# tartarughina/S-BLAS

Hardware: AMD Instinct MI355X
Metric: SpMM GFLOP/s (2*nnz*N/t), CSR x dense N=64, fp64 (higher is better)
Workload: dtype f64; 1 GPU; SpMM method-1 (dense-B column partition), nd24k-like synthetic (M=K=72000, 399 nnz/row, band +-2000, seed 211), nnz=28728000, N=64 columns per GPU, alpha=beta=1, B = srand(211)/rand() as the reference's DenseMatrix, inputs resident in HBM; step = B->row-major staging + row-panel SpMM; rows=72000, cols=72000, nnz=28728000, n_cols_per_gpu=64, parallelism=method1-colblock x1

## Files before the change

include/sblas_hip.h:

```cpp
#ifndef SBLAS_HIP_H
#define SBLAS_HIP_H

#include <stddef.h>
#include <stdint.h>

#ifdef __cplusplus
extern "C" {
#endif

#define SBLAS_OK 0
#define SBLAS_E_INVALID 1
#define SBLAS_E_HIP 2
#define SBLAS_E_WORKSPACE 3
#define SBLAS_E_RCCL 4
#define SBLAS_E_IO 5
#define SBLAS_E_NOGPU 6

int sblas_hip_version(void);
const char *sblas_hip_error_string(int code);
int sblas_hip_device_count(void);

size_t sblas_hip_spmm_csr_f64_i32_workspace(int64_t rows, int64_t cols, int64_t nnz, int64_t n);

int sblas_hip_spmm_csr_f64_i32(int dev, void *stream,
// ... 255 lines not shown
    SBLAS_SPMM_RULE_STAGING = 0,
    SBLAS_SPMM_RULE_VERDICTS,
    SBLAS_SPMM_RULE_PANEL_ROWS,
    SBLAS_SPMM_RULE_GROUPS,
    SBLAS_SPMM_RULE_PANELS,
    SBLAS_SPMM_RULE_PLANNABLE,
    SBLAS_SPMM_RULE_TILED,
    SBLAS_SPMM_RULE_TILED_G,
    SBLAS_SPMM_RULE_W6_NH,
    SBLAS_SPMM_RULE_W6_GRID_Y,
    SBLAS_SPMM_RULE_LANES_NC,
    SBLAS_SPMM_RULE_LANES_CP,
    SBLAS_SPMM_RULE_LANES_LPE,
    SBLAS_SPMM_RULE_MFMA,
    SBLAS_SPMM_RULE_MFMA_BATCH,
    SBLAS_SPMM_RULE_MFMA_LDS_FLOOR,
    SBLAS_SPMM_RULE_FOUR_ROWS,
    SBLAS_SPMM_RULE_FOUR_ROWS_WAVES,
    SBLAS_SPMM_RULE_FOUR_ROWS_VOTED,
    SBLAS_SPMM_RULE_MERGE,
    SBLAS_SPMM_RULE_DPP_GROUPS,
    SBLAS_SPMM_RULE_DPP_PAD,
    SBLAS_SPMM_RULE_DPP_LONG,
    SBLAS_SPMM_RULE_NARROW,
    SBLAS_SPMM_RULE_ROWS8,
    SBLAS_SPMM_RULE_INTERLEAVE,
    SBLAS_SPMM_RULE_SKIP,
    SBLAS_SPMM_RULE_SPLIT_GROUPS,
    SBLAS_SPMM_RULE_FIELDS
};
int64_t sblas_spmm_rule_describe(int64_t rows, int64_t cols, int64_t nnz, int64_t ldbt, int64_t n, int64_t ncu,
                                 int caller_staged, const int64_t *plan, int64_t *out, int64_t max_out);

int sblas_host_fill_rand0to1(double *dst, int64_t count, unsigned seed);

int sblas_mm_read_info(const char *path, int32_t *rows, int32_t *cols, int32_t *nnz,
                       int32_t *is_symmetric);
int sblas_mm_read_csr(const char *path, int32_t *rowptr, int32_t *colidx, double *val);

#ifdef __cplusplus
}
#endif
#endif
```

s-blas_amd/csrc/kernels.hip:

```cpp
#include <hip/hip_runtime.h>
#include <atomic>
#include <stdint.h>
#include <algorithm>
#include <type_traits>
#include <mutex>
#include <vector>
#include "kernels.h"

namespace sblas {

constexpr int WAVE = 64;

__device__ __forceinline__ int wave_uniform(int v) { return __builtin_amdgcn_readfirstlane(v); }

__device__ __forceinline__ double readlane_f64(double v, int src_lane)
{
    int lo = __double2loint(v), hi = __double2hiint(v);
    lo = __builtin_amdgcn_readlane(lo, src_lane);
    hi = __builtin_amdgcn_readlane(hi, src_lane);
    return __hiloint2double(hi, lo);
}

constexpr int STAGE_K = 32;
template <bool RB>
__device__ __forceinline__ void stage_tile(double (*tile)[STAGE_K + 1], int64_t k0, int64_t j0, int64_t cols, int64_t n,
                                           const double *__restrict__ B, int64_t ldb, double *__restrict__ Bt,
                                           int64_t ldbt, int *__restrict__ tail, int stage_epoch)
{
    if constexpr (RB) {
        const int jl = threadIdx.x & 63, kq = threadIdx.x >> 6;
        const int64_t j = j0 + jl;
        double v[8];
#pragma unroll
        for (int u = 0; u < 8; ++u) {
            const int64_t kr = k0 + kq + 4 * u;
            v[u] = (j < n && kr < cols) ? B[kr * ldb + j] : 0.0;
        }
        bool odd = false;
#pragma unroll
        for (int u = 0; u < 8; ++u) odd |= (__double2hiint(v[u]) & 0x7ff00000) == 0x7ff00000;
// ... 577 lines not shown
                 "v_fmac_f64_dpp %[c3], %[gv], v[110:111] row_newbcast:" #K1 " row_mask:0xf bank_mask:0xf\n\t"       \
                 "s_waitcnt lgkmcnt(3)\n\t"                                                                          \
                 "v_fmac_f64_dpp %[c0], %[gv], v[112:113] row_newbcast:" #K2 " row_mask:0xf bank_mask:0xf\n\t"       \
                 "v_fmac_f64_dpp %[c1], %[gv], v[114:115] row_newbcast:" #K2 " row_mask:0xf bank_mask:0xf\n\t"       \
                 "s_waitcnt lgkmcnt(2)\n\t"                                                                          \
                 "v_fmac_f64_dpp %[c2], %[gv], v[116:117] row_newbcast:" #K2 " row_mask:0xf bank_mask:0xf\n\t"       \
                 "v_fmac_f64_dpp %[c3], %[gv], v[118:119] row_newbcast:" #K2 " row_mask:0xf bank_mask:0xf\n\t"       \
                 "s_waitcnt lgkmcnt(1)\n\t"                                                                          \
                 "v_fmac_f64_dpp %[c0], %[gv], v[120:121] row_newbcast:" #K3 " row_mask:0xf bank_mask:0xf\n\t"       \
                 "v_fmac_f64_dpp %[c1], %[gv], v[122:123] row_newbcast:" #K3 " row_mask:0xf bank_mask:0xf\n\t"       \
                 "s_waitcnt lgkmcnt(0)\n\t"                                                                          \
                 "v_fmac_f64_dpp %[c2], %[gv], v[124:125] row_newbcast:" #K3 " row_mask:0xf bank_mask:0xf\n\t"       \
                 "v_fmac_f64_dpp %[c3], %[gv], v[126:127] row_newbcast:" #K3 " row_mask:0xf bank_mask:0xf\n\t"       \
                 : [c0] "+v"(q0), [c1] "+v"(q1), [c2] "+v"(q2), [c3] "+v"(q3)                                        \
                 : [co] "v"(co), [lb] "v"(lb), [gv] "v"(gv)                                                          \
                 : "memory", "v92", "v93", "v94", "v95", "v96", "v97", "v98", "v99", "v100", "v101", "v102", "v103", \
                   "v104", "v105", "v106", "v107", "v108", "v109", "v110", "v111", "v112", "v113", "v114", "v115",   \
                   "v116", "v117", "v118", "v119", "v120", "v121", "v122", "v123", "v124", "v125", "v126", "v127")

__device__ __forceinline__ void dma_rows_scalar(unsigned lds_addr, unsigned voff, const char *base)
{
    asm volatile("s_mov_b32 m0, %0\n\ts_nop 0\n\tglobal_load_lds_dwordx4 %1, %2" ::"s"(lds_addr), "v"(voff), "s"(base)
                 : "memory");
}
__device__ __forceinline__ void dma_rows_vector(unsigned lds_addr, const char *addr)
{
    asm volatile("s_mov_b32 m0, %0\n\ts_nop 0\n\tglobal_load_lds_dwordx4 %1, off" ::"s"(lds_addr), "v"(addr)
                 : "memory");
}

static_assert(4 * 4 * 2 >= SPMM_MIN_PANEL_ROWS, "the workspace reserves one verdict per SPMM_MIN_PANEL_ROWS rows");


__device__ __forceinline__ void window_select6(int wc, double wv, int tile_lo, int rem, int k, unsigned zero_rel,
                                               unsigned &co, double &gv, unsigned long long &m)
{
    int glo, ghi;
    asm volatile("v_subrev_u32 %[co], %[tlo], %[wc]\n\t"
                 "v_cmp_gt_i32 %[m], %[rem], %[k]\n\t"
                 "v_cmp_gt_u32 vcc, %[tr], %[co]\n\t"
                 "v_lshlrev_b32 %[co], 9, %[co]\n\t"
                 "s_and_b64 vcc, vcc, %[m]\n\t"
                 "s_mov_b64 %[m], vcc\n\t"
                 "v_cndmask_b32 %[co], %[zr], %[co], vcc\n\t"
                 "v_cndmask_b32 %[glo], 0, %[vlo], vcc\n\t"
                 "v_cndmask_b32 %[ghi], 0, %[vhi], vcc"
                 : [co] "=&v"(co), [m] "=&s"(m), [glo] "=&v"(glo), [ghi] "=&v"(ghi)
                 : [tlo] "s"(tile_lo), [wc] "v"(wc), [rem] "v"(rem), [k] "v"(k), [zr] "v"(zero_rel),
                   [vlo] "v"(__double2loint(wv)), [vhi] "v"(__double2hiint(wv)), [tr] "n"(W2_ROWS)
                 : "vcc", "scc");
    gv = __hiloint2double(ghi, glo);
}
__device__ __forceinline__ void window_issue6(sblas_rsrc_t rc, sblas_rsrc_t rv, int idx, int &ca, double &va, int &cb,
                                              double &vb)
{
    const int idx2 = idx + 16;
    asm volatile("buffer_load_dword %0, %4, %6, 0 idxen\n\t"
                 "buffer_load_dwordx2 %1, %4, %7, 0 idxen\n\t"
                 "buffer_load_dword %2, %5, %6, 0 idxen\n\t"
                 "buffer_load_dwordx2 %3, %5, %7, 0 idxen"
                 : "=&v"(ca), "=&v"(va), "=&v"(cb), "=&v"(vb)
                 : "v"(idx), "v"(idx2), "s"(rc), "s"(rv)
                 : "memory");
}
template <int NEWER> __device__ __forceinline__ void window_wait6(int &ca, double &va, int &cb, double &vb)
{
    static_assert(NEWER == 0 || NEWER == 4 || NEWER == 8, "counts of the sixth-generation tile loop");
    if (NEWER == 4) asm volatile("s_waitcnt vmcnt(4)" : "+v"(ca), "+v"(va), "+v"(cb), "+v"(vb)::"memory");
    else if (NEWER == 8) asm volatile("s_waitcnt vmcnt(8)" : "+v"(ca), "+v"(va), "+v"(cb), "+v"(vb)::"memory");
    else asm volatile("s_waitcnt vmcnt(0)" : "+v"(ca), "+v"(va), "+v"(cb), "+v"(vb)::"memory");
}
template <int N> __device__ __forceinline__ void vm_wait6()
{
    static_assert(N == 8 || N == 12, "counts of the sixth-generation tile loop");
    if (N == 12) asm volatile("s_waitcnt vmcnt(12)" ::: "memory");
    else asm volatile("s_waitcnt vmcnt(8)" ::: "memory");
}

template <int G, int NH, bool RC>
__global__ __launch_bounds__(1024) void spmm_window6_kernel(
    int rows, int cols, int npanels, const int *__restrict__ rowptr, const int *__restrict__ colidx,
    const double *__restrict__ val, const double *__restrict__ Bt, int64_t ldbt, int n, double alpha, double beta,
    double *__restrict__ C, int64_t ldc, const int *__restrict__ tail, const int2 *__restrict__ info,
    const int *__restrict__ cls, int panel_rows, int nnz)
{
    constexpr int RW = 4 * G, RMAX = 16 * RW;
    static_assert(G == 2 || G == 3, "two or three groups per wave (the counted vmcnt waits are 4 G)");
    static_assert(NH == 1 || NH == 2, "one or two 64-column halves per workgroup");
    static_assert(64 * (RMAX + 1) <= 2 * W2_TILE, "C tile must fit in the (dead) B tile buffers");
    extern __shared__ __attribute__((aligned(16))) double smem[];
    double *zero_row = smem + 2 * W2_TILE;
    int *sm_i = reinterpret_cast<int *>(smem + 2 * W2_TILE + 64);

    const int panel = xcd_contiguous_panel(blockIdx.x, npanels);
    if (!owns_window(tail, cls, panel)) return;
    const int2 span = info[panel];

    const int tid = threadIdx.x;
    const int lane = tid & 63;
    const int wave = wave_uniform(tid >> 6);
    const int row0 = panel * panel_rows;
    const int col0 = blockIdx.y * (64 * NH);
    const unsigned ld32 = (unsigned)ldbt;
    const int t_lo = span.x / W2_ROWS, t_hi = span.y / W2_ROWS;
    const bool loader = wave >= 12;
    const bool active = !loader && wave * RW < panel_rows;

    if (tid < 64) zero_row[tid] = 0.0;
    if (tid == 0) sm_i[0] = 0;

    double acc[NH][G][4];
#pragma unroll
    for (int h = 0; h < NH; ++h)
#pragma unroll
        for (int g = 0; g < G; ++g)
#pragma unroll
            for (int j = 0; j < 4; ++j) acc[h][g][j] = 0.0;

    const unsigned ldb8 = ld32 * 8u;
    const unsigned piece_off = (unsigned)(col0 + ((lane & 31) << 1)) * 8u;
    const unsigned pair_off = (unsigned)(lane >> 5) * ldb8 + piece_off;
    const char *bt_bytes = reinterpret_cast<const char *>(Bt);
    int dummy = 0;
    auto dma_part = [&](int t, int h, int buf) {
        const int lw = wave - 12;
        const int r0 = t * W2_ROWS + lw * W2_LROWS;
        const unsigned lds0 = (unsigned)wave_uniform((int)((unsigned)(uintptr_t)(smem + buf * W2_TILE) + (unsigned)lw * (unsigned)(W2_LROWS * 512)));
        const unsigned hoff = (unsigned)h * 512u;
        if (r0 + W2_LROWS - 1 <= cols) {
            const char *p = bt_bytes + (size_t)((unsigned)r0 * ldb8) + hoff;
#pragma unroll
            for (int i = 0; i < W2_LROWS / 2; ++i) dma_rows_scalar(lds0 + i * 1024u, pair_off, p + (size_t)(2u * i) * ldb8);
        } else {
#pragma unroll
            for (int i = 0; i < W2_LROWS / 2; ++i) {
                const unsigned brow = (unsigned)min(r0 + 2 * i + (lane >> 5), cols);
                dma_rows_vector(lds0 + i * 1024u, bt_bytes + (size_t)(brow * ldb8 + piece_off + hoff));
            }
        }
    };

    if (loader) dma_part(t_lo, 0, 0);

    const int k = lane & 15, q = lane >> 4;
    const int wrow = min(row0 + wave * RW, rows);
    const int wstart = wave_uniform(rowptr[wrow]);
    const sblas_rsrc_t rc = make_rsrc(colidx + wstart, 4u, (unsigned)(nnz - wstart));
    const sblas_rsrc_t rv = make_rsrc(val + wstart, 8u, (unsigned)(nnz - wstart));
    int cur[G], end[G];
#pragma unroll
    for (int g = 0; g < G; ++g) {
        const int rr = wave * RW + 4 * g + q;
        const int row = row0 + rr;
        cur[g] = end[g] = 0;
        if (rr < panel_rows && row < rows) {
            cur[g] = rowptr[row] - wstart;
            end[g] = rowptr[row + 1] - wstart;
        }
    }
    unsigned long long viol = 0ull;
    int wca[G], wcb[G];
    double wva[G], wvb[G];
    unsigned s_coA[G], s_coB[G];
    double s_gvA[G], s_gvB[G];
    int s_take[G], s_mx[G];
    bool replay[G];
#pragma unroll
    for (int g = 0; g < G; ++g) {
        s_coA[g] = s_coB[g] = 0u;
        s_gvA[g] = s_gvB[g] = 0.0;
        s_take[g] = s_mx[g] = 0;
        replay[g] = false;
    }
#pragma unroll
    for (int g = 0; g < G; ++g) window_issue6(rc, rv, cur[g] + k, wca[g], wva[g], wcb[g], wvb[g]);
    asm volatile("s_waitcnt vmcnt(0)" ::: "memory");
    __syncthreads();
    int step = 0;
    for (int t = t_lo; t <= t_hi; ++t) {
        const int tile_lo = t * W2_ROWS;
        auto half = [&](auto hc) {
            constexpr int h = decltype(hc)::value;
            const int cbuf = step & 1;
            if (loader) {
                if (h + 1 < NH) dma_part(t, h + 1, cbuf ^ 1);
                else if (t < t_hi) dma_part(t + 1, 0, cbuf ^ 1);
            }
            const unsigned tile_base = (unsigned)(uintptr_t)(smem + cbuf * W2_TILE);
            const unsigned lb = tile_base + (unsigned)k * 16u;
            const unsigned zero_rel = (unsigned)(uintptr_t)zero_row - tile_base;
            auto visit = [&](auto gc) {
                constexpr int g = decltype(gc)::value;
                if (h == 0) window_wait6<NH == 1 ? 4 * (G - 1) : 4 * (G - 1 - g)>(wca[g], wva[g], wcb[g], wvb[g]);
                else if (replay[g]) window_wait6<0>(wca[g], wva[g], wcb[g], wvb[g]);
                double &q0 = acc[h][g][0], &q1 = acc[h][g][1], &q2 = acc[h][g][2], &q3 = acc[h][g][3];
                int lc = cur[g];
                bool full = h == 0 || replay[g];
                for (;;) {
                    unsigned coA, coB;
                    double gvA, gvB;
                    int take, mx;
                    if (full) {
                        const int rem = end[g] - lc;
                        unsigned long long mA, mB;
                        window_select6(wca[g], wva[g], tile_lo, rem, k, zero_rel, coA, gvA, mA);
                        window_select6(wcb[g], wvb[g], tile_lo, rem - 16, k, zero_rel, coB, gvB, mB);
                        const unsigned fa = q < 2 ? (unsigned)mA : (unsigned)(mA >> 32);
                        const unsigned fb = q < 2 ? (unsigned)mB : (unsigned)(mB >> 32);
                        const int sh = (q & 1) * 16;
                        take = __popc((fa >> sh) & 0xffffu) + __popc((fb >> sh) & 0xffffu);
                        viol |= mA ^ __builtin_amdgcn_ballot_w64(k < take);
                        viol |= mB ^ __builtin_amdgcn_ballot_w64(k + 16 < take);
                        mx = max(max(__builtin_amdgcn_readlane(take, 0), __builtin_amdgcn_readlane(take, 16)),
                                 max(__builtin_amdgcn_readlane(take, 32), __builtin_amdgcn_readlane(take, 48)));
                        if (NH > 1 && h == 0) {
                            s_coA[g] = coA, s_coB[g] = coB, s_gvA[g] = gvA, s_gvB[g] = gvB, s_take[g] = take, s_mx[g] = mx;
// ... 5 lines not shown
                    {
                        const unsigned co = coA;
                        const double gv = gvA;
                        if (mx > 0) { SBLAS_QSTEP4(0, 1, 2, 3); }
                        if (mx > 4) { SBLAS_QSTEP4(4, 5, 6, 7); }
                        if (mx > 8) { SBLAS_QSTEP4(8, 9, 10, 11); }
                        if (mx > 12) { SBLAS_QSTEP4(12, 13, 14, 15); }
                    }
                    if (mx > 16) {
                        const unsigned co = coB;
                        const double gv = gvB;
                        SBLAS_QSTEP4(0, 1, 2, 3);
                        if (mx > 20) { SBLAS_QSTEP4(4, 5, 6, 7); }
                        if (mx > 24) { SBLAS_QSTEP4(8, 9, 10, 11); }
                        if (mx > 28) { SBLAS_QSTEP4(12, 13, 14, 15); }
                    }
                    asm volatile("s_setprio 0" ::: "memory");
                    lc += take;
                    const bool more = take >= 32 && lc < end[g];
                    if (__builtin_expect(__builtin_amdgcn_ballot_w64(more) == 0ull, 1)) break;
                    if (NH > 1 && h == 0) replay[g] = true;
                    window_issue6(rc, rv, lc + k, wca[g], wva[g], wcb[g], wvb[g]);
                    window_wait6<0>(wca[g], wva[g], wcb[g], wvb[g]);
                    full = true;
                }
                if (h == NH - 1) {
                    cur[g] = lc;
                    if (NH > 1) replay[g] = false;
                    window_issue6(rc, rv, cur[g] + k, wca[g], wva[g], wcb[g], wvb[g]);
                } else if (replay[g]) {
                    window_issue6(rc, rv, cur[g] + k, wca[g], wva[g], wcb[g], wvb[g]);
                }
            };
            if (active) {
                visit(std::integral_constant<int, 0>{});
                visit(std::integral_constant<int, 1>{});
                if constexpr (G > 2) visit(std::integral_constant<int, 2>{});
            }
            if (loader) asm volatile("s_waitcnt vmcnt(0)" : "+v"(dummy)::"memory");
            __syncthreads();
            ++step;
        };
        half(std::integral_constant<int, 0>{});
        if constexpr (NH > 1) half(std::integral_constant<int, 1>{});
    }
#pragma unroll
    for (int g = 0; g < G; ++g) window_wait6<0>(wca[g], wva[g], wcb[g], wvb[g]);
    int bad = viol != 0ull ? 1 : 0;
#pragma unroll
    for (int g = 0; g < G; ++g)
        if (__builtin_amdgcn_ballot_w64(cur[g] < end[g]) != 0ull) bad = 1;
    if (bad && lane == 0) atomicOr(&sm_i[0], 1);
    __syncthreads();
    const bool fell_back = sm_i[0] != 0;
    if (tid == 0 && blockIdx.y == 0) atomicAdd(&g_panel_stats[fell_back ? 2 : 0], 1ull);

    double *ctile = smem;
    const int nrows = min(panel_rows, rows - row0);
#pragma unroll
    for (int h = 0; h < NH; ++h) {
        const int colh = col0 + 64 * h;
        if (fell_back) {
            const unsigned lane_off = (unsigned)(colh + lane);
#pragma unroll
            for (int g = 0; g < G; ++g)
#pragma unroll
                for (int j = 0; j < 4; ++j) {
                    const int rr = wave * RW + 4 * g + j;
                    const int row = row0 + rr;
                    int a = 0, b = 0;
// ... 1574 lines not shown
```

s-blas_amd/csrc/spmm_rule.cpp:

```cpp
#include <stdint.h>
#include <stdio.h>
#include <stdlib.h>
#include <string.h>
#include <algorithm>
#include <atomic>
#include <mutex>
#include "../../include/sblas_hip.h"
#include "kernels.h"

namespace sblas {

static Options g_options;
static std::atomic<bool> g_options_loaded{false};
static std::mutex g_options_mu;
static void options_parse(Options &o)
{
    o = Options{};
    const char *e;
    if ((e = getenv("SBLAS_SPMM_VARIANT")) && *e) {
        if (!strcmp(e, "dpp")) o.spmm_variant = SPMM_VARIANT_DIRECT_DPP;
        else if (!strcmp(e, "rows")) o.spmm_variant = SPMM_VARIANT_DIRECT_ROWS;
        else if (!strcmp(e, "lanes")) o.spmm_variant = SPMM_VARIANT_LANES;
        else if (!strcmp(e, "merge")) o.spmm_variant = SPMM_VARIANT_DIRECT_MERGE;
        else if (!strcmp(e, "mfma")) o.spmm_variant = SPMM_VARIANT_MFMA;
        else if (!strcmp(e, "nomfma")) o.spmm_variant = SPMM_VARIANT_NO_MFMA;
    }
    if ((e = getenv("SBLAS_SPMV_VARIANT")) && *e && strcmp(e, "auto")) {
        strncpy(o.spmv_variant, e, sizeof o.spmv_variant - 1);
    }
    if ((e = getenv("SBLAS_SPMM_MIN_LDBT")) && *e) o.tier16 = o.tier32 = atoi(e) < 64;
    if ((e = getenv("SBLAS_SPMM_MAX_BT_BYTES")) && *e) {
        const unsigned long long v = strtoull(e, nullptr, 10);
        if (v >= 4096 && v < 0xffffffffull) o.max_bt_bytes = v;
    }
    if ((e = getenv("SBLAS_DIRECT_LDS")) && *e) o.direct_lds = atoi(e);
    if ((e = getenv("SBLAS_DIRECT_MERGE")) && *e) o.direct_merge = atoi(e);
    if ((e = getenv("SBLAS_STAGE_RANGE")) && *e) o.stage_range = atoi(e);
    if ((e = getenv("SBLAS_DIRECT_MAP")) && *e) o.direct_map = !strcmp(e, "interleave") ? 1 : !strcmp(e, "contiguous") ? 0 : -1;
    if ((e = getenv("SBLAS_ROWS8_MIN_AVG")) && *e) o.rows8_min_avg = atof(e);
    if ((e = getenv("SBLAS_WINDOW_DENSITY")) && *e) o.window_density = (float)atof(e);
    if ((e = getenv("SBLAS_SPMM_PANEL_ROWS")) && *e) {
// ... 277 lines not shown
        pv.n_window = (long)plan[SBLAS_SPMM_RULE_PLAN_N_WINDOW], pv.n_direct = (long)plan[SBLAS_SPMM_RULE_PLAN_N_DIRECT];
        pv.n_mfma_w = (long)plan[SBLAS_SPMM_RULE_PLAN_N_MFMA_W], pv.n_mfma_d = (long)plan[SBLAS_SPMM_RULE_PLAN_N_MFMA_D];
        pv.merge = plan[SBLAS_SPMM_RULE_PLAN_MERGE] != 0, pv.four_rows = plan[SBLAS_SPMM_RULE_PLAN_FOUR_ROWS] != 0;
        pv.n_split = plan[SBLAS_SPMM_RULE_PLAN_N_SPLIT];
        pv.info_rows = (int)plan[SBLAS_SPMM_RULE_PLAN_PANEL_ROWS], pv.groups = (int)plan[SBLAS_SPMM_RULE_PLAN_GROUPS];
    }
    bool again = false;
    const sblas::SpmmStep st = sblas::step_rule((int)rows, (int)cols, nnz, ldbt, plan ? &pv : nullptr, sblas::SpmmStep(),
                                                caller_staged != 0, (int)ncu, again);
    const sblas::SpmmStage2 d = sblas::spmm_stage2(st, (int)rows, (int)cols, nnz, (int)n);
    int64_t f[SBLAS_SPMM_RULE_FIELDS] = {0};
    f[SBLAS_SPMM_RULE_STAGING] = st.staging, f[SBLAS_SPMM_RULE_VERDICTS] = st.verdicts;
    f[SBLAS_SPMM_RULE_PANEL_ROWS] = st.info_rows, f[SBLAS_SPMM_RULE_GROUPS] = st.groups;
    f[SBLAS_SPMM_RULE_PANELS] = st.npanels, f[SBLAS_SPMM_RULE_PLANNABLE] = st.plannable;
    f[SBLAS_SPMM_RULE_TILED] = d.tiled, f[SBLAS_SPMM_RULE_TILED_G] = d.tiled ? d.g : 0;
    f[SBLAS_SPMM_RULE_W6_NH] = d.nh, f[SBLAS_SPMM_RULE_W6_GRID_Y] = d.grid_y;
    f[SBLAS_SPMM_RULE_LANES_NC] = d.nc, f[SBLAS_SPMM_RULE_LANES_CP] = d.cp, f[SBLAS_SPMM_RULE_LANES_LPE] = d.lpe;
    f[SBLAS_SPMM_RULE_MFMA] = d.mfma;
    f[SBLAS_SPMM_RULE_MFMA_BATCH] = d.mfma ? d.mfma_batch : 0;
    f[SBLAS_SPMM_RULE_MFMA_LDS_FLOOR] = d.mfma ? (int64_t)d.mfma_lds_floor : 0;
    f[SBLAS_SPMM_RULE_FOUR_ROWS] = d.four_rows;
    f[SBLAS_SPMM_RULE_FOUR_ROWS_WAVES] = d.four_rows ? d.rows_waves : 0;
    f[SBLAS_SPMM_RULE_FOUR_ROWS_VOTED] = d.voted;
    f[SBLAS_SPMM_RULE_MERGE] = d.merge;
    f[SBLAS_SPMM_RULE_DPP_GROUPS] = d.dpp;
    f[SBLAS_SPMM_RULE_DPP_PAD] = d.dpp ? (int64_t)d.dpp_pad : 0;
    f[SBLAS_SPMM_RULE_DPP_LONG] = d.dpp ? d.dpp_long : 0;
    f[SBLAS_SPMM_RULE_NARROW] = d.narrow, f[SBLAS_SPMM_RULE_ROWS8] = d.rows8;
    f[SBLAS_SPMM_RULE_INTERLEAVE] = d.interleave;
    f[SBLAS_SPMM_RULE_SKIP] = d.skip, f[SBLAS_SPMM_RULE_SPLIT_GROUPS] = d.skip ? d.split_groups : 0;
    for (int64_t k = 0; out && k < SBLAS_SPMM_RULE_FIELDS && k < max_out; ++k) out[k] = f[k];
    return SBLAS_SPMM_RULE_FIELDS;
}
```

s-blas_amd/python/sblas_amd/__init__.py:

```python
import ctypes as C
import os

import numpy as np

_PKG = os.path.dirname(os.path.abspath(__file__))
_ROOT = os.path.normpath(os.path.join(_PKG, "..", ".."))
LIB_PATH = os.environ.get("SBLAS_LIB_PATH") or os.path.join(_ROOT, "lib", "libsblas_hip.so")

EXPORTS = [
    "sblas_hip_version", "sblas_hip_error_string", "sblas_hip_device_count",
    "sblas_hip_spmm_csr_f64_i32_workspace", "sblas_hip_spmm_csr_f64_i32", "sblas_hip_spmm_ldbt",
    "sblas_hip_dense_to_rowmajor_f64", "sblas_hip_spmm_csr_rowmajorB_f64_i32",
    "sblas_hip_debug_spmm_panel_stats", "sblas_hip_debug_reload_env",
    "sblas_hip_debug_spmm_kernel_events", "sblas_hip_debug_spmm_last_kernel_ms", "sblas_hip_spmv_csr_f64_i32", "sblas_hip_axpby_f64",
    "sblas_hip_comm_get", "sblas_hip_comm_release_all", "sblas_hip_allreduce_sum_f64",
    "sblas_hip_merge_rowblocks_f64", "sblas_hip_merge_rowblocks_local_f64",
    "sblas_find_row_of_nnz", "sblas_partition_nnz", "sblas_partition_dense",
    "sblas_mm_read_info", "sblas_mm_read_csr", "sblas_host_fill_rand0to1",
    "sblas_hip_spmm_csr_workspace", "sblas_hip_spmm_csr", "sblas_hip_spmv_csr", "sblas_hip_axpby",
    "sblas_hip_allreduce_sum", "sblas_hip_merge_rowblocks", "sblas_partition_nnz_i64",
    "sblas_hip_debug_validate_csr_i32",
    "sblas_hip_spmm_plan_create", "sblas_hip_spmm_plan_destroy", "sblas_hip_spmm_plan_info", "sblas_hip_spmm_csr_f64_i32_planned",
    "sblas_hip_spmv_plan_create", "sblas_hip_spmv_plan_destroy", "sblas_hip_spmv_plan_info", "sblas_hip_spmv_csr_f64_i32_planned",
    "sblas_spmv_plan_classify",
    "sblas_hip_spmm_csr_ordered", "sblas_hip_spmm_csr_ordered_f64_i32_planned", "sblas_hip_merge_rowblocks_ordered",
    "sblas_hip_spmm_plan_create_split", "sblas_hip_spmm_plan_split_info", "sblas_spmm_split_classify",
    "sblas_spmm_rule_describe",
    "sblas_hip_csr_transpose_workspace", "sblas_hip_csr_transpose_f64_i32", "sblas_hip_gather_f64",
    "sblas_hip_transpose_plan_create", "sblas_hip_transpose_plan_update_values", "sblas_hip_transpose_plan_info",
    "sblas_hip_transpose_plan_csc", "sblas_hip_transpose_plan_destroy", "sblas_hip_spmv_csr_t_f64_i32_planned",
    "sblas_hip_spmm_csr_t_f64_i32_planned",
    "sblas_hip_coo_to_csr_workspace", "sblas_hip_coo_to_csr_f64_i32", "sblas_hip_coo_plan_create", "sblas_hip_coo_plan_info",
    "sblas_hip_coo_plan_csr", "sblas_hip_coo_plan_assemble", "sblas_hip_coo_plan_destroy",
    "sblas_hip_sddmm_csr_workspace", "sblas_hip_sddmm_csr_f64_i32",
    "sblas_hip_csr_softmax_workspace", "sblas_hip_csr_softmax_f64_i32", "sblas_hip_csr_softmax_backward_f64_i32",
    "sblas_hip_csr_attention_workspace", "sblas_hip_csr_attention_f64_i32", "sblas_hip_csr_attention_backward_f64_i32",
    "sblas_hip_spgemm_limits", "sblas_hip_spgemm_classify", "sblas_hip_spgemm_group_width", "sblas_hip_spgemm_check_nnz",
    "sblas_hip_spgemm_plan_create", "sblas_hip_spgemm_plan_info", "sblas_hip_spgemm_plan_csr", "sblas_hip_spgemm_plan_numeric",
    "sblas_hip_spgemm_plan_destroy",
    "sblas_hip_sptrsv_limits", "sblas_sptrsv_levels", "sblas_sptrsv_schedule",
    "sblas_hip_sptrsv_plan_create", "sblas_hip_sptrsv_plan_info", "sblas_hip_sptrsv_plan_order", "sblas_hip_sptrsv_plan_destroy",
    "sblas_hip_sptrsv_f64_i32_planned", "sblas_hip_sptrsm_f64_i32_planned",
]


class SblasError(RuntimeError):
    pass


_lib = None


def lib():
    global _lib
    if _lib is not None:
        return _lib
    if not os.path.exists(LIB_PATH):
        raise SblasError("libsblas_hip.so not built (%s): run __graft_entry__.build() / make -C s-blas_amd" % LIB_PATH)
    import torch
    L = C.CDLL(LIB_PATH)
    i64, i32, f64, vp, sz = C.c_int64, C.c_int32, C.c_double, C.c_void_p, C.c_size_t
    L.sblas_hip_version.restype = C.c_int
    L.sblas_hip_error_string.restype = C.c_char_p
    L.sblas_hip_error_string.argtypes = [C.c_int]
    L.sblas_hip_device_count.restype = C.c_int
    L.sblas_hip_spmm_ldbt.restype = i64
    L.sblas_hip_spmm_ldbt.argtypes = [i64]
    L.sblas_hip_spmm_csr_f64_i32_workspace.restype = sz
    L.sblas_hip_spmm_csr_f64_i32_workspace.argtypes = [i64, i64, i64, i64]
    L.sblas_hip_spmm_csr_f64_i32.restype = C.c_int
    L.sblas_hip_spmm_csr_f64_i32.argtypes = [C.c_int, vp, i64, i64, i64, vp, vp, vp, vp, i64, i64, f64, f64, vp, i64, vp, sz]
    L.sblas_hip_debug_validate_csr_i32.restype = C.c_int
    L.sblas_hip_debug_validate_csr_i32.argtypes = [C.c_int, vp, i64, i64, i64, vp, vp]
    L.sblas_hip_spmm_plan_create.restype = C.c_int
    L.sblas_hip_spmm_plan_create.argtypes = [C.c_int, vp, i64, i64, i64, vp, vp, i64, C.POINTER(vp)]
    L.sblas_hip_spmm_plan_create_split.restype = C.c_int
    L.sblas_hip_spmm_plan_create_split.argtypes = [C.c_int, vp, i64, i64, i64, vp, vp, i64, i64, i64, C.POINTER(vp)]
    L.sblas_hip_spmm_plan_split_info.restype = C.c_int
    L.sblas_hip_spmm_plan_split_info.argtypes = [vp, C.POINTER(i64)]
    L.sblas_spmm_split_classify.restype = i64
    L.sblas_spmm_split_classify.argtypes = [vp, i64, i64, i64, i64, vp, i64, vp, i64]
    L.sblas_spmm_rule_describe.restype = i64
    L.sblas_spmm_rule_describe.argtypes = [i64, i64, i64, i64, i64, i64, C.c_int, vp, vp, i64]
    L.sblas_hip_spmm_plan_destroy.restype = C.c_int
    L.sblas_hip_spmm_plan_destroy.argtypes = [vp]
    L.sblas_hip_spmm_plan_info.restype = C.c_int
    L.sblas_hip_spmm_plan_info.argtypes = [vp, C.POINTER(i64)]
    L.sblas_hip_spmm_csr_f64_i32_planned.restype = C.c_int
    L.sblas_hip_spmm_csr_f64_i32_planned.argtypes = [vp, C.c_int, vp, i64, i64, i64, vp, vp, vp, vp, i64, i64, f64, f64, vp, i64, vp, sz]
    L.sblas_hip_spmv_plan_create.restype = C.c_int
    L.sblas_hip_spmv_plan_create.argtypes = [C.c_int, vp, i64, i64, i64, vp, vp, C.POINTER(vp)]
    L.sblas_hip_spmv_plan_destroy.restype = C.c_int
    L.sblas_hip_spmv_plan_destroy.argtypes = [vp]
    L.sblas_hip_spmv_plan_info.restype = C.c_int
    L.sblas_hip_spmv_plan_info.argtypes = [vp, C.POINTER(i64)]
    L.sblas_hip_spmv_csr_f64_i32_planned.restype = C.c_int
    L.sblas_hip_spmv_csr_f64_i32_planned.argtypes = [vp, C.c_int, vp, i64, i64, i64, vp, vp, vp, vp, f64, f64, vp]
    L.sblas_spmv_plan_classify.restype = i64
    L.sblas_spmv_plan_classify.argtypes = [vp, i64, i64, i64, i64, vp, i64]
    L.sblas_hip_dense_to_rowmajor_f64.restype = C.c_int
    L.sblas_hip_dense_to_rowmajor_f64.argtypes = [C.c_int, vp, i64, i64, vp, i64, vp, i64]
    L.sblas_hip_spmm_csr_rowmajorB_f64_i32.restype = C.c_int
    L.sblas_hip_spmm_csr_rowmajorB_f64_i32.argtypes = [C.c_int, vp, i64, i64, i64, vp, vp, vp, vp, i64, i64, f64, f64, vp, i64]
    L.sblas_hip_debug_reload_env.restype = C.c_int
    L.sblas_hip_debug_reload_env.argtypes = []
    L.sblas_hip_debug_spmm_panel_stats.restype = C.c_int
    L.sblas_hip_debug_spmm_panel_stats.argtypes = [C.POINTER(C.c_uint64), C.c_int]
    L.sblas_hip_debug_spmm_kernel_events.restype = C.c_int
    L.sblas_hip_debug_spmm_kernel_events.argtypes = [C.c_int]
    L.sblas_hip_debug_spmm_last_kernel_ms.restype = C.c_int
    L.sblas_hip_debug_spmm_last_kernel_ms.argtypes = [C.POINTER(C.c_float)]
    L.sblas_hip_spmv_csr_f64_i32.restype = C.c_int
    L.sblas_hip_spmv_csr_f64_i32.argtypes = [C.c_int, vp, i64, i64, i64, vp, vp, vp, vp, f64, f64, vp]
    L.sblas_hip_axpby_f64.restype = C.c_int
    L.sblas_hip_axpby_f64.argtypes = [C.c_int, vp, i64, f64, vp, f64, vp]
    L.sblas_hip_comm_get.restype = C.c_int
# ... 321 lines not shown

def sptrsv_schedule(widths, mode="auto", chain_rows=0):
    widths = np.ascontiguousarray(widths, np.int64)
    L = len(widths)
    kind = np.zeros(max(L, 1), np.uint8)
    first = np.zeros(L + 1, np.int64)
    n = C.c_int64()
    check(lib().sblas_sptrsv_schedule(L, widths.ctypes.data, _sptrsv_mode(mode), int(chain_rows), kind.ctypes.data,
                                      first.ctypes.data, C.byref(n)), "sblas_sptrsv_schedule")
    return kind[:n.value].copy(), first[:n.value + 1].copy()


def partition_dense(first_order, n_gpu, i_gpu):
    o, d = C.c_int64(), C.c_int64()
    check(lib().sblas_partition_dense(first_order, n_gpu, i_gpu, C.byref(o), C.byref(d)), "sblas_partition_dense")
    return o.value, d.value


def _dev_ptr(t, dtype, what):
    import torch
    if not isinstance(t, torch.Tensor) or not t.is_cuda:
        raise SblasError("%s must be a GPU tensor (no CPU path exists)" % what)
    if t.dtype != dtype or not t.is_contiguous():
        raise SblasError("%s must be a contiguous %s tensor" % (what, dtype))
    return t.data_ptr()


def _stream(stream=None):
    import torch
    s = stream if stream is not None else torch.cuda.current_stream()
    return C.c_void_p(s.cuda_stream)


def spmm_workspace_bytes(rows, cols, nnz, n):
    return int(lib().sblas_hip_spmm_csr_f64_i32_workspace(rows, cols, nnz, n))


def spmm(rows, cols, rowptr, colidx, val, B, ldb, n, alpha, beta, Cmat, ldc, workspace, stream=None, c_offset=0):
    import torch
    nnz = int(colidx.numel())
    rc = lib().sblas_hip_spmm_csr_f64_i32(
        -1, _stream(stream), rows, cols, nnz,
        _dev_ptr(rowptr, torch.int32, "rowptr"), _dev_ptr(colidx, torch.int32, "colidx") if nnz else None,
        _dev_ptr(val, torch.float64, "val") if nnz else None,
        _dev_ptr(B, torch.float64, "B") if cols else None, ldb, n, alpha, beta,
        _dev_ptr(Cmat, torch.float64, "C") + 8 * c_offset, ldc,
        _dev_ptr(workspace, torch.float64, "workspace") if workspace is not None and workspace.numel() else None,
        workspace.numel() * 8 if workspace is not None else 0)
    check(rc, "sblas_hip_spmm_csr_f64_i32")


class SpmmPlan:

    def __init__(self, rows, cols, rowptr, colidx, n, stream=None, split=False, split_min=0, piece=0):
        import torch
        self.rows, self.cols, self.n, self.rowptr, self.colidx = rows, cols, n, rowptr, colidx
        self.nnz = int(colidx.numel())
        h = C.c_void_p()
        args = (-1, _stream(stream), rows, cols, self.nnz, _dev_ptr(rowptr, torch.int32, "rowptr"),
                _dev_ptr(colidx, torch.int32, "colidx") if self.nnz else None, n)
        if split:
            check(lib().sblas_hip_spmm_plan_create_split(*args, split_min, piece, C.byref(h)), "sblas_hip_spmm_plan_create_split")
        else:
            check(lib().sblas_hip_spmm_plan_create(*args, C.byref(h)), "sblas_hip_spmm_plan_create")
        self.handle = h

# ... 1090 lines not shown
```

Baseline: 15050 GFLOP/s.

## Add aligned three-chunk ring buffer for colidx/val window loads in window6 kernel

For the single-half (NH==1) window6 kernel, colidx/val loads move from a sliding window at cur+k to a three-chunk ring aligned to the val pointer's 128-byte phase. Chunks already consumed are shifted in registers and only the newly needed chunks are fetched. The aim is cache-line-aligned, non-redundant nonzero loads across B tiles. The cost is a wider per-tile select and mask path (three selects per group), plus a possible refetch loop with a full vmcnt(0) wait. A host replay function is added to validate the ring logic.

```diff
diff --git a/include/sblas_hip.h b/include/sblas_hip.h
--- a/include/sblas_hip.h
+++ b/include/sblas_hip.h
@@ -311,6 +311,9 @@
 int64_t sblas_spmm_rule_describe(int64_t rows, int64_t cols, int64_t nnz, int64_t ldbt, int64_t n, int64_t ncu,
                                  int caller_staged, const int64_t *plan, int64_t *out, int64_t max_out);
 
+int64_t sblas_window_ring_replay(int64_t nnz, int64_t phase, int64_t cur, int64_t end, const int64_t *takes, int64_t ntakes,
+                                 int64_t *out, int64_t max_out, int64_t *stats);
+
 int sblas_host_fill_rand0to1(double *dst, int64_t count, unsigned seed);
 
 int sblas_mm_read_info(const char *path, int32_t *rows, int32_t *cols, int32_t *nnz,
diff --git a/s-blas_amd/csrc/kernels.hip b/s-blas_amd/csrc/kernels.hip
--- a/s-blas_amd/csrc/kernels.hip
+++ b/s-blas_amd/csrc/kernels.hip
@@ -6,6 +6,7 @@
 #include <mutex>
 #include <vector>
 #include "kernels.h"
+#include "window_ring.h"
 
 namespace sblas {
 
@@ -649,25 +650,29 @@
 static_assert(4 * 4 * 2 >= SPMM_MIN_PANEL_ROWS, "the workspace reserves one verdict per SPMM_MIN_PANEL_ROWS rows");
 
 
+#define SBLAS_SELECT6(CMP)                                                                                            \
+    asm volatile("v_subrev_u32 %[co], %[tlo], %[wc]\n\t" CMP " %[m], %[rem], %[k]\n\t"                               \
+                 "v_cmp_gt_u32 vcc, %[tr], %[co]\n\t"                                                                 \
+                 "v_lshlrev_b32 %[co], 9, %[co]\n\t"                                                                  \
+                 "s_and_b64 vcc, vcc, %[m]\n\t"                                                                       \
+                 "s_mov_b64 %[m], vcc\n\t"                                                                            \
+                 "v_cndmask_b32 %[co], %[zr], %[co], vcc\n\t"                                                         \
+                 "v_cndmask_b32 %[glo], 0, %[vlo], vcc\n\t"                                                           \
+                 "v_cndmask_b32 %[ghi], 0, %[vhi], vcc"                                                                \
+                 : [co] "=&v"(co), [m] "=&s"(m), [glo] "=&v"(glo), [ghi] "=&v"(ghi)                                    \
+                 : [tlo] "s"(tile_lo), [wc] "v"(wc), [rem] "v"(rem), [k] "v"(k), [zr] "v"(zero_rel),                   \
+                   [vlo] "v"(__double2loint(wv)), [vhi] "v"(__double2hiint(wv)), [tr] "n"(W2_ROWS)                     \
+                 : "vcc", "scc")
+template <bool RING = false>
 __device__ __forceinline__ void window_select6(int wc, double wv, int tile_lo, int rem, int k, unsigned zero_rel,
                                                unsigned &co, double &gv, unsigned long long &m)
 {
     int glo, ghi;
-    asm volatile("v_subrev_u32 %[co], %[tlo], %[wc]\n\t"
-                 "v_cmp_gt_i32 %[m], %[rem], %[k]\n\t"
-                 "v_cmp_gt_u32 vcc, %[tr], %[co]\n\t"
-                 "v_lshlrev_b32 %[co], 9, %[co]\n\t"
-                 "s_and_b64 vcc, vcc, %[m]\n\t"
-                 "s_mov_b64 %[m], vcc\n\t"
-                 "v_cndmask_b32 %[co], %[zr], %[co], vcc\n\t"
-                 "v_cndmask_b32 %[glo], 0, %[vlo], vcc\n\t"
-                 "v_cndmask_b32 %[ghi], 0, %[vhi], vcc"
-                 : [co] "=&v"(co), [m] "=&s"(m), [glo] "=&v"(glo), [ghi] "=&v"(ghi)
-                 : [tlo] "s"(tile_lo), [wc] "v"(wc), [rem] "v"(rem), [k] "v"(k), [zr] "v"(zero_rel),
-                   [vlo] "v"(__double2loint(wv)), [vhi] "v"(__double2hiint(wv)), [tr] "n"(W2_ROWS)
-                 : "vcc", "scc");
+    if constexpr (RING) SBLAS_SELECT6("v_cmp_gt_u32");
+    else SBLAS_SELECT6("v_cmp_gt_i32");
     gv = __hiloint2double(ghi, glo);
 }
+#undef SBLAS_SELECT6
 __device__ __forceinline__ void window_issue6(sblas_rsrc_t rc, sblas_rsrc_t rv, int idx, int &ca, double &va, int &cb,
                                               double &vb)
 {
@@ -694,6 +699,55 @@
     else asm volatile("s_waitcnt vmcnt(8)" ::: "memory");
 }
 
+__device__ __forceinline__ void ring_issue_all(sblas_rsrc_t rc, sblas_rsrc_t rv, int e0, int &c0, double &v0, int &c1,
+                                               double &v1, int &c2, double &v2)
+{
+    const int e1 = e0 + ring::CHUNK, e2 = e0 + 2 * ring::CHUNK;
+    asm volatile("buffer_load_dword %0, %6, %9, 0 idxen\n\t"
+                 "buffer_load_dwordx2 %1, %6, %10, 0 idxen\n\t"
+                 "buffer_load_dword %2, %7, %9, 0 idxen\n\t"
+                 "buffer_load_dwordx2 %3, %7, %10, 0 idxen\n\t"
+                 "buffer_load_dword %4, %8, %9, 0 idxen\n\t"
+                 "buffer_load_dwordx2 %5, %8, %10, 0 idxen"
+                 : "=&v"(c0), "=&v"(v0), "=&v"(c1), "=&v"(v1), "=&v"(c2), "=&v"(v2)
+                 : "v"(e0), "v"(e1), "v"(e2), "s"(rc), "s"(rv)
+                 : "memory");
+}
+__device__ __forceinline__ void ring_wait_all(int &c0, double &v0, int &c1, double &v1, int &c2, double &v2)
+{
+    asm volatile("s_waitcnt vmcnt(0)" : "+v"(c0), "+v"(v0), "+v"(c1), "+v"(v1), "+v"(c2), "+v"(v2)::"memory");
+}
+__device__ __forceinline__ void ring_advance(sblas_rsrc_t rc, sblas_rsrc_t rv, int e1, int e2, int n, int &c0, double &v0,
+                                             int &c1, double &v1, int &c2, double &v2)
+{
+    unsigned long long all;
+    asm volatile("s_mov_b64 %[all], exec\n\t"
+                 "v_cmp_lt_u32 vcc, 0, %[n]\n\t"
+                 "s_mov_b64 exec, vcc\n\t"
+                 "v_mov_b32 %[c0], %[c1]\n\t"
+                 "v_mov_b64 %[v0], %[v1]\n\t"
+                 "v_cmp_eq_u32 vcc, 1, %[n]\n\t"
+                 "s_mov_b64 exec, vcc\n\t"
+                 "v_mov_b32 %[c1], %[c2]\n\t"
+                 "v_mov_b64 %[v1], %[v2]\n\t"
+                 "s_mov_b64 exec, %[all]\n\t"
+                 "v_cmp_eq_u32 vcc, 2, %[n]\n\t"
+                 "s_mov_b64 exec, vcc\n\t"
+                 "v_mov_b32 %[c0], %[c2]\n\t"
+                 "v_mov_b64 %[v0], %[v2]\n\t"
+                 "buffer_load_dword %[c1], %[e1], %[rc], 0 idxen\n\t"
+                 "buffer_load_dwordx2 %[v1], %[e1], %[rv], 0 idxen\n\t"
+                 "s_mov_b64 exec, %[all]\n\t"
+                 "v_cmp_lt_u32 vcc, 0, %[n]\n\t"
+                 "s_mov_b64 exec, vcc\n\t"
+                 "buffer_load_dword %[c2], %[e2], %[rc], 0 idxen\n\t"
+                 "buffer_load_dwordx2 %[v2], %[e2], %[rv], 0 idxen\n\t"
+                 "s_mov_b64 exec, %[all]"
+                 : [all] "=&s"(all), [c0] "+v"(c0), [v0] "+v"(v0), [c1] "+v"(c1), [v1] "+v"(v1), [c2] "+v"(c2), [v2] "+v"(v2)
+                 : [e1] "v"(e1), [e2] "v"(e2), [n] "v"(n), [rc] "s"(rc), [rv] "s"(rv)
+                 : "memory", "vcc");
+}
+
 template <int G, int NH, bool RC>
 __global__ __launch_bounds__(1024) void spmm_window6_kernel(
     int rows, int cols, int npanels, const int *__restrict__ rowptr, const int *__restrict__ colidx,
@@ -702,6 +756,7 @@
     const int *__restrict__ cls, int panel_rows, int nnz)
 {
     constexpr int RW = 4 * G, RMAX = 16 * RW;
+    constexpr bool RING = NH == 1;
     static_assert(G == 2 || G == 3, "two or three groups per wave (the counted vmcnt waits are 4 G)");
     static_assert(NH == 1 || NH == 2, "one or two 64-column halves per workgroup");
     static_assert(64 * (RMAX + 1) <= 2 * W2_TILE, "C tile must fit in the (dead) B tile buffers");
@@ -761,9 +816,10 @@
 
     const int k = lane & 15, q = lane >> 4;
     const int wrow = min(row0 + wave * RW, rows);
-    const int wstart = wave_uniform(rowptr[wrow]);
+    const int wstart = RING ? 0 : wave_uniform(rowptr[wrow]);
     const sblas_rsrc_t rc = make_rsrc(colidx + wstart, 4u, (unsigned)(nnz - wstart));
     const sblas_rsrc_t rv = make_rsrc(val + wstart, 8u, (unsigned)(nnz - wstart));
+    const int phase = wave_uniform(ring::phase((uint64_t)(uintptr_t)val));
     int cur[G], end[G];
 #pragma unroll
     for (int g = 0; g < G; ++g) {
@@ -778,6 +834,8 @@
     unsigned long long viol = 0ull;
     int wca[G], wcb[G];
     double wva[G], wvb[G];
+    int wc0[G], re0[G];
+    double wv0[G];
     unsigned s_coA[G], s_coB[G];
     double s_gvA[G], s_gvB[G];
     int s_take[G], s_mx[G];
@@ -790,7 +848,19 @@
         replay[g] = false;
     }
 #pragma unroll
-    for (int g = 0; g < G; ++g) window_issue6(rc, rv, cur[g] + k, wca[g], wva[g], wcb[g], wvb[g]);
+    for (int g = 0; g < G; ++g) {
+        if constexpr (RING) {
+            re0[g] = ring::r0_entry(cur[g], phase, k);
+            ring_issue_all(rc, rv, re0[g], wc0[g], wv0[g], wca[g], wva[g], wcb[g], wvb[g]);
+        } else {
+            wc0[g] = re0[g] = 0, wv0[g] = 0.0;
+            window_issue6(rc, rv, cur[g] + k, wca[g], wva[g], wcb[g], wvb[g]);
+        }
+    }
+    if constexpr (RING) {
+#pragma unroll
+        for (int g = 0; g < G; ++g) ring_wait_all(wc0[g], wv0[g], wca[g], wva[g], wcb[g], wvb[g]);
+    }
     asm volatile("s_waitcnt vmcnt(0)" ::: "memory");
     __syncthreads();
     int step = 0;
@@ -798,7 +868,7 @@
         const int tile_lo = t * W2_ROWS;
         auto half = [&](auto hc) {
             constexpr int h = decltype(hc)::value;
-            const int cbuf = step & 1;
+            const int cbuf = NH == 1 ? (t - t_lo) & 1 : step & 1;
             if (loader) {
                 if (h + 1 < NH) dma_part(t, h + 1, cbuf ^ 1);
                 else if (t < t_hi) dma_part(t + 1, 0, cbuf ^ 1);
@@ -870,10 +940,84 @@
                     window_issue6(rc, rv, cur[g] + k, wca[g], wva[g], wcb[g], wvb[g]);
                 }
             };
+            auto visit_ring = [&](auto gc) {
+                constexpr int g = decltype(gc)::value;
+                window_wait6<4 * (G - 1)>(wca[g], wva[g], wcb[g], wvb[g]);
+                double &q0 = acc[0][g][0], &q1 = acc[0][g][1], &q2 = acc[0][g][2], &q3 = acc[0][g][3];
+                int lc = cur[g];
+                int off, take;
+                for (;;) {
+                    const int len = end[g] - lc;
+                    const int d0 = re0[g] - lc;
+                    unsigned co0, co1, co2;
+                    double gv0, gv1, gv2;
+                    unsigned long long m0, m1, m2;
+                    window_select6<true>(wc0[g], wv0[g], tile_lo, len, d0, zero_rel, co0, gv0, m0);
+                    window_select6<true>(wca[g], wva[g], tile_lo, len, d0 + ring::CHUNK, zero_rel, co1, gv1, m1);
+                    window_select6<true>(wcb[g], wvb[g], tile_lo, len, d0 + 2 * ring::CHUNK, zero_rel, co2, gv2, m2);
+                    const int sh = (q & 1) * 16;
+                    const unsigned f0 = q < 2 ? (unsigned)m0 : (unsigned)(m0 >> 32);
+                    const unsigned f1 = q < 2 ? (unsigned)m1 : (unsigned)(m1 >> 32);
+                    const unsigned f2 = q < 2 ? (unsigned)m2 : (unsigned)(m2 >> 32);
+                    take = __popc((f0 >> sh) & 0xffffu) + __popc((f1 >> sh) & 0xffffu) + __popc((f2 >> sh) & 0xffffu);
+                    off = k - d0;
+                    viol |= m0 ^ __builtin_amdgcn_ballot_w64((unsigned)d0 < (unsigned)take);
+                    viol |= m1 ^ __builtin_amdgcn_ballot_w64((unsigned)(d0 + ring::CHUNK) < (unsigned)take);
+                    viol |= m2 ^ __builtin_amdgcn_ballot_w64((unsigned)(d0 + 2 * ring::CHUNK) < (unsigned)take);
+                    auto rows_or = [](unsigned long long m) {
+                        const unsigned u = (unsigned)m | (unsigned)(m >> 32);
+                        return (u | (u >> 16)) & 0xffffu;
+                    };
+                    const unsigned u0 = rows_or(m0), u1 = rows_or(m1), u2 = rows_or(m2);
+                    asm volatile("s_setprio 1" ::: "memory");
+                    if (u0) {
+                        const unsigned co = co0;
+                        const double gv = gv0;
+                        if (u0 & 0x000fu) { SBLAS_QSTEP4(0, 1, 2, 3); }
+                        if (u0 & 0x00f0u) { SBLAS_QSTEP4(4, 5, 6, 7); }
+                        if (u0 & 0x0f00u) { SBLAS_QSTEP4(8, 9, 10, 11); }
+                        if (u0 & 0xf000u) { SBLAS_QSTEP4(12, 13, 14, 15); }
+                    }
+                    if (u1) {
+                        const unsigned co = co1;
+                        const double gv = gv1;
+                        if (u1 & 0x000fu) { SBLAS_QSTEP4(0, 1, 2, 3); }
+                        if (u1 & 0x00f0u) { SBLAS_QSTEP4(4, 5, 6, 7); }
+                        if (u1 & 0x0f00u) { SBLAS_QSTEP4(8, 9, 10, 11); }
+                        if (u1 & 0xf000u) { SBLAS_QSTEP4(12, 13, 14, 15); }
+                    }
+                    if (u2) {
+                        const unsigned co = co2;
+                        const double gv = gv2;
+                        if (u2 & 0x000fu) { SBLAS_QSTEP4(0, 1, 2, 3); }
+                        if (u2 & 0x00f0u) { SBLAS_QSTEP4(4, 5, 6, 7); }
+                        if (u2 & 0x0f00u) { SBLAS_QSTEP4(8, 9, 10, 11); }
+                        if (u2 & 0xf000u) { SBLAS_QSTEP4(12, 13, 14, 15); }
+                    }
+                    asm volatile("s_setprio 0" ::: "memory");
+                    lc += take;
+                    const bool more = ring::overflow(off, take, lc, end[g]);
+                    if (__builtin_expect(__builtin_amdgcn_ballot_w64(more) == 0ull, 1)) break;
+                    re0[g] += (off + take) & -ring::CHUNK;
+                    ring_issue_all(rc, rv, re0[g], wc0[g], wv0[g], wca[g], wva[g], wcb[g], wvb[g]);
+                    ring_wait_all(wc0[g], wv0[g], wca[g], wva[g], wcb[g], wvb[g]);
+                }
+                cur[g] = lc;
+                const int n = ring::crossed(off, take);
+                re0[g] += ring::CHUNK * n;
+                ring_advance(rc, rv, re0[g] + ring::CHUNK, re0[g] + 2 * ring::CHUNK, n, wc0[g], wv0[g], wca[g], wva[g], wcb[g],
+                             wvb[g]);
+            };
             if (active) {
-                visit(std::integral_constant<int, 0>{});
-                visit(std::integral_constant<int, 1>{});
-                if constexpr (G > 2) visit(std::integral_constant<int, 2>{});
+                if constexpr (RING) {
+                    visit_ring(std::integral_constant<int, 0>{});
+                    visit_ring(std::integral_constant<int, 1>{});
+                    if constexpr (G > 2) visit_ring(std::integral_constant<int, 2>{});
+                } else {
+                    visit(std::integral_constant<int, 0>{});
+                    visit(std::integral_constant<int, 1>{});
+                    if constexpr (G > 2) visit(std::integral_constant<int, 2>{});
+                }
             }
             if (loader) asm volatile("s_waitcnt vmcnt(0)" : "+v"(dummy)::"memory");
             __syncthreads();
diff --git a/s-blas_amd/csrc/spmm_rule.cpp b/s-blas_amd/csrc/spmm_rule.cpp
--- a/s-blas_amd/csrc/spmm_rule.cpp
+++ b/s-blas_amd/csrc/spmm_rule.cpp
@@ -7,6 +7,7 @@
 #include <mutex>
 #include "../../include/sblas_hip.h"
 #include "kernels.h"
+#include "window_ring.h"
 
 namespace sblas {
 
@@ -350,3 +351,61 @@
     for (int64_t k = 0; out && k < SBLAS_SPMM_RULE_FIELDS && k < max_out; ++k) out[k] = f[k];
     return SBLAS_SPMM_RULE_FIELDS;
 }
+
+extern "C" int64_t sblas_window_ring_replay(int64_t nnz, int64_t phase, int64_t cur, int64_t end, const int64_t *takes,
+                                            int64_t ntakes, int64_t *out, int64_t max_out, int64_t *stats)
+{
+    namespace R = sblas::ring;
+    if (nnz < 0 || nnz > INT32_MAX || phase < 0 || phase >= R::CHUNK || cur < 0 || cur > end || end > nnz || ntakes < 0 ||
+        (ntakes && !takes) || max_out < 0 || (max_out && !out))
+        return -1;
+    const int p = (int)phase, row_end = (int)end;
+    int64_t held[R::CHUNKS][R::CHUNK];
+    int64_t st[4] = {0, 0, 0, 0}, delivered = 0;
+    int lc = (int)cur, b = 0;
+    auto fetch = [&](int j, int c) {
+        for (int k = 0; k < R::CHUNK; ++k) {
+            const int64_t e = (int64_t)R::chunk_first(c, p) + k;
+            held[j][k] = e >= 0 && e < nnz ? e : -1;
+        }
+    };
+    auto fetch_ring = [&]() {
+        b = R::chunk_of(lc, p);
+        for (int j = 0; j < R::CHUNKS; ++j) fetch(j, b + j);
+    };
+    fetch_ring();
+    for (int64_t i = 0; i < ntakes; ++i) {
+        if (takes[i] < 0 || takes[i] > row_end - lc) return -1;
+        const int tile_end = lc + (int)takes[i];
+        for (;;) {
+            const int off = lc - R::chunk_first(b, p);
+            int take = 0;
+            for (int j = 0; j < R::CHUNKS; ++j)
+                for (int k = 0; k < R::CHUNK; ++k) {
+                    const int e = R::r0_entry(R::chunk_first(b, p), p, k) + R::CHUNK * j;
+                    const int64_t h = held[j][k];
+                    const bool in_tile = !(h >= tile_end && h < row_end);
+                    if (!(R::in_row(e, lc, row_end) && in_tile)) continue;
+                    if (h != e || e < 0 || e >= nnz) ++st[3];
+                    if (delivered < max_out) out[delivered] = h;
+                    ++delivered, ++take;
+                }
+            lc += take;
+            if (!R::overflow(off, take, lc, row_end)) {
+                const int n = R::crossed(off, take);
+                int64_t was[R::CHUNKS][R::CHUNK];
+                memcpy(was, held, sizeof held);
+                for (int j = 0; j < R::CHUNKS; ++j) memcpy(held[j], was[R::move_source(j, n)], sizeof held[j]);
+                for (int j = 1; j < R::CHUNKS; ++j)
+                    if (R::fetched(j, n)) fetch(j, R::fetch_chunk(j, b, n)), ++st[0];
+                b += n;
+                st[2] += n == 2;
+                break;
+            }
+            fetch_ring();
+            ++st[1];
+        }
+    }
+    for (int k = 0; stats && k < 4; ++k) stats[k] = st[k];
+    return delivered;
+}
diff --git a/s-blas_amd/csrc/window_ring.h b/s-blas_amd/csrc/window_ring.h
--- /dev/null
+++ b/s-blas_amd/csrc/window_ring.h
@@ -0,0 +1,38 @@
+#pragma once
+#include <cstdint>
+
+#if defined(__HIPCC__) || defined(__CUDACC__)
+#define SBLAS_RING_FN __host__ __device__ inline
+#else
+#define SBLAS_RING_FN inline
+#endif
+
+namespace sblas {
+namespace ring {
+
+constexpr int CHUNK = 16;
+constexpr int CHUNKS = 3;
+constexpr int SPAN = CHUNK * CHUNKS;
+
+SBLAS_RING_FN int phase(uint64_t val_address) { return (int)((val_address >> 3) & 15u); }
+SBLAS_RING_FN int chunk_of(int e, int p) { return (e + p) >> 4; }
+SBLAS_RING_FN int chunk_first(int c, int p) { return CHUNK * c - p; }
+SBLAS_RING_FN int r0_entry(int cur, int p, int k) { return chunk_first(chunk_of(cur, p), p) + k; }
+SBLAS_RING_FN bool in_row(int e, int cur, int end) { return (unsigned)(e - cur) < (unsigned)(end - cur); }
+SBLAS_RING_FN int crossed(int off, int take)
+{
+    const int n = (off + take) >> 4;
+    return n < 2 ? n : 2;
+}
+SBLAS_RING_FN bool overflow(int off, int take, int cur_after, int end) { return off + take >= SPAN && cur_after < end; }
+SBLAS_RING_FN int move_source(int j, int n)
+{
+    if (j == 0) return n;
+    if (j == 1) return n == 1 ? 2 : 1;
+    return 2;
+}
+SBLAS_RING_FN bool fetched(int j, int n) { return j == 1 ? n == 2 : (j == 2 && n >= 1); }
+SBLAS_RING_FN int fetch_chunk(int j, int b, int n) { return b + n + j; }
+
+}
+}
diff --git a/s-blas_amd/python/sblas_amd/__init__.py b/s-blas_amd/python/sblas_amd/__init__.py
--- a/s-blas_amd/python/sblas_amd/__init__.py
+++ b/s-blas_amd/python/sblas_amd/__init__.py
@@ -25,7 +25,7 @@
     "sblas_spmv_plan_classify",
     "sblas_hip_spmm_csr_ordered", "sblas_hip_spmm_csr_ordered_f64_i32_planned", "sblas_hip_merge_rowblocks_ordered",
     "sblas_hip_spmm_plan_create_split", "sblas_hip_spmm_plan_split_info", "sblas_spmm_split_classify",
-    "sblas_spmm_rule_describe",
+    "sblas_spmm_rule_describe", "sblas_window_ring_replay",
     "sblas_hip_csr_transpose_workspace", "sblas_hip_csr_transpose_f64_i32", "sblas_hip_gather_f64",
     "sblas_hip_transpose_plan_create", "sblas_hip_transpose_plan_update_values", "sblas_hip_transpose_plan_info",
     "sblas_hip_transpose_plan_csc", "sblas_hip_transpose_plan_destroy", "sblas_hip_spmv_csr_t_f64_i32_planned",
@@ -82,6 +82,8 @@
     L.sblas_spmm_split_classify.argtypes = [vp, i64, i64, i64, i64, vp, i64, vp, i64]
     L.sblas_spmm_rule_describe.restype = i64
     L.sblas_spmm_rule_describe.argtypes = [i64, i64, i64, i64, i64, i64, C.c_int, vp, vp, i64]
+    L.sblas_window_ring_replay.restype = i64
+    L.sblas_window_ring_replay.argtypes = [i64, i64, i64, i64, vp, i64, vp, i64, vp]
     L.sblas_hip_spmm_plan_destroy.restype = C.c_int
     L.sblas_hip_spmm_plan_destroy.argtypes = [vp]
     L.sblas_hip_spmm_plan_info.restype = C.c_int
@@ -469,6 +471,19 @@
     return C.c_void_p(s.cuda_stream)
 
 
+def window_ring_replay(nnz, phase, cur, end, takes):
+    t = np.ascontiguousarray(takes, np.int64)
+    out = np.full(max(int(end - cur), 1) + 64, -2, np.int64)
+    st = np.zeros(4, np.int64)
+    got = lib().sblas_window_ring_replay(nnz, phase, cur, end, t.ctypes.data if t.size else None, t.size, out.ctypes.data,
+                                         out.size, st.ctypes.data)
+    if got < 0:
+        raise SblasError("sblas_window_ring_replay refused its arguments")
+    if got > out.size:
+        raise SblasError("sblas_window_ring_replay delivered %d entries of a row of %d" % (got, end - cur))
+    return out[:got].tolist(), dict(fetched=int(st[0]), refetches=int(st[1]), crossed_two=int(st[2]), wrongly_valid=int(st[3]))
+
+
 def spmm_workspace_bytes(rows, cols, nnz, n):
     return int(lib().sblas_hip_spmm_csr_f64_i32_workspace(rows, cols, nnz, n))
 
```

Measured after the change: 12350 GFLOP/s. 18.0% lower.
